# Ignaciagothe/tda-eeg-audio

Hardware: AMD Instinct MI355X
Metric: windows/sec end-to-end (dist->Rips H0/H1->Wasserstein), 47-ch EEG (higher is better)
Workload: dtype f64; 1 GPU; configs[4]+configs[2]: 1416 recordings x 5 bands x 15 selected windows = 106200 (EEG 47x250 f64, audio 250 f64) window pairs per pass, the whole job; per pair corr->dist->Rips H0/H1 (EEG 47 pts), tau per recording-band, Takens dim 3 sub 2 + Rips (audio, 23..123 pts over the bands), Wasserstein H0+H1, features, per-recording reductions; one all-gather of the (1416, 5x48) rows per pass; windows_per_pass=106200, windows_per_gpu_per_pass=106200, input_bytes_per_gpu=10195200000, batches_per_pass=1, windows_per_batch=106200, parallelism=recordings dealt over 1 rank(s), one all-gather per pass, batches_in_flight=3, hip_graph=True, batches_rerun_with_full_ladder=0

## Files before the change

### tda_eeg_audio_amd/csrc/rips.hip

```cpp
#include "common.h"
#include "corr_dist_dev.h"
#include <stdlib.h>

#ifndef CLOUD_NB
#define CLOUD_NB 8192
#endif
#ifndef NARROW_NT
#define NARROW_NT 512
#endif
#ifndef NARROW_WAVES
#define NARROW_WAVES 6
#endif
#if defined(TDA_PROFILE) && !defined(TDA_PROFILE_STOPS_ONLY)
#define NARROW_NB (NARROW_NT == 384 ? 1536 : 1024)
#else
#define NARROW_NB (NARROW_NT == 384 ? 1536 : 2048)
#endif
#define NARROW_EMAX 7626
#define NT_MAX 512
#define RANK_NONE 0x7fffu

#ifdef TDA_PROFILE
__device__ unsigned long long g_prof[48];
#ifdef TDA_PROFILE_STOPS_ONLY
#define PROF_BEGIN() do {} while (0)
#define PROF_RESUME() do {} while (0)
#define PROF_MARK(i) do {} while (0)
#define PROF_COUNT(i, v) do {} while (0)
#define PROF_FLUSH() do {} while (0)
#else
__shared__ unsigned long long prof_lds[48];
#define PROF_BEGIN()                                                       \
    if (threadIdx.x < 48) prof_lds[threadIdx.x] = 0ull;                    \
    __syncthreads();                                                       \
    unsigned long long prof_t0 = clock64()
#define PROF_RESUME() unsigned long long prof_t0 = clock64()
#define PROF_MARK(i)                                                       \
    do {                                                                   \
        unsigned long long prof_t1 = clock64();                            \
        if (threadIdx.x == 0) prof_lds[i] += prof_t1 - prof_t0;            \
        prof_t0 = prof_t1;                                                 \
    } while (0)
#define PROF_COUNT(i, v) do { if (threadIdx.x == 0) prof_lds[i] += (unsigned long long)(v); } while (0)
#define PROF_FLUSH()                                                       \
    do {                                                                   \
        __syncthreads();                                                   \
        if (threadIdx.x < 48 && prof_lds[threadIdx.x]) atomicAdd(&g_prof[threadIdx.x], prof_lds[threadIdx.x]); \
    } while (0)
#endif
__device__ int g_stop_after;
extern "C" __attribute__((visibility("default"))) int tda_profile_stop_after(int n)
{
    return hipMemcpyToSymbol(HIP_SYMBOL(g_stop_after), &n, sizeof(int)) != hipSuccess;
}
#define PROF_STOP(n, cleanup) do { if (g_stop_after == (n)) { cleanup; return; } } while (0)
#define PROF_STOPC(n, cleanup) do { if (g_stop_after == (n) + 100 * prof_chunk) { cleanup; return; } } while (0)
extern "C" __attribute__((visibility("default"))) int tda_profile_read(unsigned long long* out, int reset)
{
    if (hipMemcpyFromSymbol(out, HIP_SYMBOL(g_prof), sizeof(unsigned long long) * 48) != hipSuccess) return 1;
    if (reset) {
        unsigned long long z[48] = {0};
        if (hipMemcpyToSymbol(HIP_SYMBOL(g_prof), z, sizeof(z)) != hipSuccess) return 1;
    }
    return 0;
}
#else
#define PROF_BEGIN() do {} while (0)
#define PROF_RESUME() do {} while (0)
#define PROF_MARK(i) do {} while (0)
#define PROF_COUNT(i, v) do {} while (0)
#define PROF_FLUSH() do {} while (0)
// ... 203 lines not shown
#pragma unroll 4
    for (int e = tid; e < E; e += NT) {
        const u32 b = rank[e];
        u32 r = RANK_NONE;
        if (b != 0xffffu) {
            const u32 k = key32[e];
            const int lo = b ? (int)cur16[b - 1] : 0, hi = (int)cur16[b];
            int c = 0;
            for (int j = lo; j < hi; ++j) {
                const u32 m = members[j];
                const u32 km = key32[m];
                c += (km < k || (km == k && m < (u32)e)) ? 1 : 0;
            }
            r = (u32)(lo + c);
        }
        rank[e] = (u16)r;
    }
    __syncthreads();
#pragma unroll 4
    for (int e = tid; e < E; e += NT) {
        const u32 r = rank[e];
        if (r != RANK_NONE) {
            ord[r] = (u16)edge_ab(e);
            if (WANT_KEYS) skey[r] = key32[e];
        }
    }
    __syncthreads();
    return Ev;
}

#if defined(TDA_PROFILE) && !defined(TDA_PROFILE_STOPS_ONLY)
#define NARROW_LDS ((160 * 1024 / 3 / 1280) * 1280 - 384)
#else
#define NARROW_LDS ((160 * 1024 / 3 / 1280) * 1280)
#endif
#define NARROW_PMAX 124
#define NARROW_DIM 3
#ifdef TDA_DEBUG_PTS
#define NL_GUARD 16
#else
#define NL_GUARD 0
#endif
#define NL_A16(x) (((x) + 15) & ~15)
struct NL {
    static constexpr int E = NARROW_EMAX;
    static constexpr int RANK = 0;
    static constexpr int PSI = NL_A16(2 * E) + NL_GUARD;
    static constexpr int MEMBERS = NL_A16(4 * E);
    static constexpr int CURSOR = NL_A16(MEMBERS + 2 * E);
    static constexpr int RSCR = CURSOR + 2 * NARROW_NB;
    static constexpr int TOTAL = NARROW_LDS;
    static constexpr int AUX = TOTAL - NL_GUARD - NL_A16(NARROW_PMAX * NARROW_DIM * 8);
    static constexpr int MISC = AUX - NL_GUARD - NL_A16(8752 + 8 * 32);
    static constexpr int REGION = MISC - NL_GUARD - PSI;
    static_assert(RSCR + 720 <= AUX - NL_GUARD, "the ranking arrays must end in front of the points");
    static_assert(MEMBERS >= 4 * (E + 1) && CURSOR >= MEMBERS + 2 * (E + 3), "room for the walk's padding (rank_edges_narrow)");
    static_assert(REGION >= 2 * E + 8 * 512, "the first chunks must fit: class vectors of 2 NT ranks next to the whole of ord");
};

template <int NT, int NB>
__device__ __forceinline__ int rank_edges_narrow(const u32* key32, int E, u32 teff, u32 kmin, u16* members, u32* cursor, int* wsum,
                                                 u16* rank, u16* ord)
{
    static_assert(NB % (2 * NT) == 0, "every thread scans whole words");
    static_assert(NB <= 0x8000, "bucket indices are parked in 16 bits, 0xffff = beyond the threshold");
    constexpr int WPT = NB / NT / 2;
    constexpr int EPT = 2 * ((NARROW_EMAX + 2 * NT - 1) / (2 * NT));
    const int tid = threadIdx.x, lane = tid & 63, wave = tid >> 6;
    Bucketer bk;
    bk.dmin = sortable_f32(kmin);
    bk.top = (float)(NB - 1);
    bk.scale = bk.top / (sortable_f32(teff) - bk.dmin);
    for (int i = tid; i < NB / 2; i += NT) cursor[i] = 0u;
    __syncthreads();
    u32 rk[EPT / 2];
#pragma unroll
    for (int i = 0; i < EPT; ++i) {
        const int e = tid + i * NT;
        u32 b = 0xffffu;
        if (e < E) {
            const u32 k = key32[e];
            if (k <= teff) { b = (u32)bk(k); atomicAdd(&cursor[b >> 1], 1u << (16 * (b & 1))); }
        }
        if (i & 1) rk[i >> 1] |= b << 16; else rk[i >> 1] = b;
    }
    __syncthreads();
    {
        u32 w[WPT];
        int s = 0;
#pragma unroll
        for (int i = 0; i < WPT; ++i) {
            const u32 x = cursor[tid * WPT + i];
            const int c0 = (int)(x & 0xffffu), c1 = (int)(x >> 16);
            w[i] = (u32)s | ((u32)(s + c0) << 16);
            s += c0 + c1;
        }
        const int incl = wave_incl_scan_i32(s);
        if (lane == 63) wsum[wave] = incl;
        __syncthreads();
        int basep = incl - s;
        for (int q = 0; q < wave; ++q) basep += wsum[q];
        const u32 add = (u32)basep * 0x00010001u;
#pragma unroll
        for (int i = 0; i < WPT; ++i) cursor[tid * WPT + i] = w[i] + add;
        if (tid == NT - 1) {
            const int total = basep + s;
            members[total] = (u16)NARROW_EMAX; members[total + 1] = (u16)NARROW_EMAX; members[total + 2] = (u16)NARROW_EMAX;
            const_cast<u32*>(key32)[NARROW_EMAX] = 0xffffffffu;
        }
    }
    __syncthreads();
#pragma unroll
    for (int i = 0; i < EPT; ++i) {
        const u32 b = i & 1 ? rk[i >> 1] >> 16 : rk[i >> 1] & 0xffffu;
        if (b != 0xffffu) {
            const int sh = 16 * (int)(b & 1u);
            const u32 old = atomicAdd(&cursor[b >> 1], 1u << sh);
            members[(old >> sh) & 0xffffu] = (u16)(tid + i * NT);
        }
    }
    __syncthreads();
    const u16* cur16 = reinterpret_cast<const u16*>(cursor);
    const int Ev = uni((int)cur16[NB - 1]);
#pragma unroll
    for (int i = 0; i < EPT; ++i) {
        const u32 e = (u32)(tid + i * NT);
        const u32 b = i & 1 ? rk[i >> 1] >> 16 : rk[i >> 1] & 0xffffu;
        u32 r = RANK_NONE;
        if (b != 0xffffu) {
            const u32 k = key32[e];
            const u64 me = ((u64)k << 32) | e;
            const int lo = b ? (int)cur16[b - 1] : 0, hi = (int)cur16[b];
            int c = 0;
            for (int j = lo; j < hi; j += 4) {
                u32 m[4], km[4];
#pragma unroll
                for (int t = 0; t < 4; ++t) m[t] = (u32)members[j + t];
#pragma unroll
                for (int t = 0; t < 4; ++t) km[t] = key32[m[t]];
#pragma unroll
                for (int t = 0; t < 4; ++t) c += ((((u64)km[t] << 32) | m[t]) < me) ? 1 : 0;
            }
            r = (u32)(lo + c);
        }
        if (i & 1) rk[i >> 1] = (rk[i >> 1] & 0xffffu) | (r << 16); else rk[i >> 1] = (rk[i >> 1] & 0xffff0000u) | r;
    }
    __syncthreads();
#pragma unroll
    for (int i = 0; i < EPT; ++i) {
        const int e = tid + i * NT;
        if (e < E) {
            const u32 r = i & 1 ? rk[i >> 1] >> 16 : rk[i >> 1] & 0xffffu;
            rank[e] = (u16)r;
            if (r != RANK_NONE) ord[r] = (u16)edge_ab(e);
        }
    }
    __syncthreads();
    return Ev;
}

struct RipsOut {
    double* h0; int h0_cap; int* h0_cnt;
    double* h1; int h1_cap; int* h1_cnt;
    int* status;
    int* retry_list = nullptr;
};

struct RipsLayout {
    int off_members;
    int off_rank, off_ord, off_aux, off_misc;
    int total;
    int off_psi, psi_bytes, off_cursor, off_rscr;
    int guard[5], n_guard;
};

#define TDA_WIN_LDS_GUARD 0x100
#ifndef TDA_SOLO_PRIO
#define TDA_SOLO_PRIO 3
#endif
#define TDA_SOLO_BEGIN() __builtin_amdgcn_s_setprio(TDA_SOLO_PRIO)
#define TDA_SOLO_END() __builtin_amdgcn_s_setprio(0)

#define TDA_POLL_LIMIT (1 << 16)
#ifndef TDA_TURN_SLEEP
#define TDA_TURN_SLEEP 4
#endif
#ifdef TDA_DEBUG_PTS
__device__ int g_fault;
extern "C" __attribute__((visibility("default"))) int tda_debug_inject(int what)
{
    return hipMemcpyToSymbol(HIP_SYMBOL(g_fault), &what, sizeof(int)) != hipSuccess;
}
#define TDA_FAULT(n) (g_fault == (n))
#else
#define TDA_FAULT(n) false
#endif
#ifdef TDA_DEBUG_PTS
#define GUARD_BYTES 16
__device__ __forceinline__ void guard_write(unsigned char* smem, const RipsLayout& L)
{
    if ((int)threadIdx.x < 4 * L.n_guard) reinterpret_cast<u32*>(smem + L.guard[threadIdx.x >> 2] - GUARD_BYTES)[threadIdx.x & 3] = 0xC0FFEE00u + threadIdx.x;
    __syncthreads();
}
__device__ __forceinline__ int guard_check(unsigned char* smem, const RipsLayout& L)
{
    __syncthreads();
    bool bad = false;
    if ((int)threadIdx.x < 4 * L.n_guard) bad = reinterpret_cast<u32*>(smem + L.guard[threadIdx.x >> 2] - GUARD_BYTES)[threadIdx.x & 3] != 0xC0FFEE00u + threadIdx.x;
    return __syncthreads_or(bad ? 1 : 0) ? TDA_WIN_LDS_GUARD : 0;
}
#else
#define GUARD_BYTES 0
__device__ __forceinline__ void guard_write(unsigned char*, const RipsLayout&) {}
__device__ __forceinline__ int guard_check(unsigned char*, const RipsLayout&) { return 0; }
#endif

#define MISC_COMP 0
#define MISC_CAND 512
#define MISC_WV (512 + 128)
#define MISC_MIN (512 + 192)
#define MISC_DONE (512 + 208)
#define MISC_SORTCNT (512 + 224)
#define MISC_SHARED (MISC_DONE + NT_MAX)
#define MISC_CKEY (MISC_SHARED + 96)
#define MISC_LIST MISC_CKEY
#define MISC_LIST_BYTES (4 * NT_MAX + 1280)
#define MISC_ADJ (MISC_LIST + MISC_LIST_BYTES)
#define MISC_ADJC (MISC_ADJ + 128 * 16)
#define MISC_BRANK (MISC_ADJC + 128 * 16)
#define MISC_BYTES(ncls) (MISC_BRANK + 8 * (ncls))

template <int NT, int NVW, int W, typename WT, bool NARROW, class KEYFN>
__device__ __forceinline__ void rips_sweep(int n, int E, int Ev, const u16* rank, const u16* ord, Psi<W, WT>* psi, int psi_bytes,
                           unsigned char* misc, KEYFN keyfn, double* h0, int h0_cap, double* h1, int h1_cap,
                           int& out_k0, int& out_k1, int& out_status)
{
    static_assert(!NARROW || W == 1, "the narrow layout is the point-cloud first pass");
    int psi_cap = 0;
    const int tid0 = threadIdx.x;
    const int lane0 = tid0 & 63, wave = uni(tid0 >> 6);
    int* brank = reinterpret_cast<int*>(misc + MISC_BRANK);
    u64* cand = reinterpret_cast<u64*>(misc + MISC_CAND);
    unsigned char* done = misc + MISC_DONE;
    SweepShared* shared = reinterpret_cast<SweepShared*>(misc + MISC_SHARED);
    u64* adj = reinterpret_cast<u64*>(misc + MISC_ADJ);
    constexpr int WB = 8 * (int)sizeof(WT);
    float* bkey = reinterpret_cast<float*>(misc + MISC_BRANK + 4 * WB * W);
    u64* adjc = reinterpret_cast<u64*>(misc + MISC_ADJC);

    if constexpr (!NARROW) for (int e = tid0; e < E; e += NT) psi[e] = pzero<W, WT>();
    for (int i = tid0; i < WB * W; i += NT) { brank[i] = -1; bkey[i] = 0.f; }
    for (int i = tid0; i < 256; i += NT) { adj[i] = 0ull; adjc[i] = 0ull; }
    if (tid0 == 0) {
        u32* lc = reinterpret_cast<u32*>(misc + MISC_MIN);
        lc[0] = 0u; lc[1] = 0xffffffffu; lc[2] = 0u;
        lc[3] = 0u;
        shared->status = 0;
    }
    if (tid0 < 16) {
        reinterpret_cast<u32*>(misc + MISC_WV)[tid0] = 0u;
        cand[tid0] = 0ull;
    }
    __syncthreads();

    WgVote vote{reinterpret_cast<u32*>(misc + MISC_WV), 0};
    WT alive[W];
#pragma unroll
    for (int c = 0; c < W; ++c) alive[c] = 0;
    int k0 = 0, k1 = 0, merges = 0, status = 0;
    int compA = lane0, compB = lane0 + 64;

    int clen = NT;
    int ordcls = 0;
    int cov_next = tid0;
#ifdef TDA_PROFILE
    int prof_rneed = 0, prof_chunk = -1;
#endif
    PROF_RESUME();
    for (int r0 = 0; r0 < Ev && !status; r0 += clen) {
        int tid = tid0;
        LAUNDER(tid);
        const int lane = tid & 63;
        clen = NT;
        PROF_MARK(15);
#ifdef TDA_PROFILE
        ++prof_chunk;
#endif
        PROF_COUNT(23, 1);
        const int r = r0 + tid;
        const bool valid = r < Ev;
        int a = 1, b = 0;
        if (valid) { const u32 pk = ord[r]; a = (int)(pk >> 8); b = (int)(pk & 255u); }
        const int tab = tri2(a) + b;
        const int slot = NARROW ? r : tab;
        if constexpr (NARROW) {
            psi_cap = (psi_bytes - 2 * (E - r0)) >> 2;
            if (r < psi_cap) psi[r] = pzero<W, WT>();
        }
        u64 M[NVW], M0[NVW];
        u64 Aj[NVW], Bj[NVW];
#pragma unroll
        for (int w = 0; w < NVW; ++w) { M[w] = 0; M0[w] = 0; Aj[w] = 0; Bj[w] = 0; }
        if (valid) {
#pragma unroll
            for (int w = 0; w < NVW; ++w) { Aj[w] = adj[2 * a + w]; Bj[w] = adj[2 * b + w]; M0[w] = Aj[w] & Bj[w]; }
        }
        {
            volatile u32* turn = reinterpret_cast<volatile u32*>(misc + MISC_MIN) + 2;
            if (wave > 0) {
                int trips = 0;
                for (;;) {
                    const u32 t = (u32)uni((int)*turn);
                    if (t >= (u32)wave) break;
                    if (++trips > TDA_POLL_LIMIT) { if (lane == 0) turn[1] = 1u; break; }
                    if (t + 1u < (u32)wave) __builtin_amdgcn_s_sleep(TDA_TURN_SLEEP); else __builtin_amdgcn_s_sleep(0);
                }
            }
            __builtin_amdgcn_fence(__ATOMIC_ACQUIRE, "workgroup");
            if (valid) {
#pragma unroll
                for (int w = 0; w < NVW; ++w) M[w] = (Aj[w] | adjc[2 * a + w]) & (Bj[w] | adjc[2 * b + w]);
                atomicOr(reinterpret_cast<unsigned long long*>(&adjc[2 * a + (b >> 6)]), 1ull << (b & 63));
                atomicOr(reinterpret_cast<unsigned long long*>(&adjc[2 * b + (a >> 6)]), 1ull << (a & 63));
            }
            LDS_ORDER();
            if (lane == 0 && !(TDA_FAULT(1) && wave == 3)) *turn = (u32)wave + 1u;
        }
        if (valid) {
            const int ta0 = tri2(a), tb0 = tri2(b);
#pragma unroll
            for (int w = 0; w < NVW; ++w) {
                u64 cc = (Aj[w] | adjc[2 * a + w]) & (Bj[w] | adjc[2 * b + w]) & ~M[w];
                while (cc) {
                    const int v0 = 64 * w + __builtin_ctzll(cc); cc &= cc - 1ull;
                    const bool ok1 = cc != 0ull; const int v1 = ok1 ? 64 * w + __builtin_ctzll(cc) : v0; cc &= cc - 1ull;
                    const int t0 = tri2(v0), t1 = tri2(v1);
                    const u32 xa0 = rank[v0 < a ? ta0 + v0 : t0 + a], xb0 = rank[v0 < b ? tb0 + v0 : t0 + b];
                    const u32 xa1 = rank[v1 < a ? ta0 + v1 : t1 + a], xb1 = rank[v1 < b ? tb0 + v1 : t1 + b];
                    if ((int)(xa0 > xb0 ? xa0 : xb0) < r) M[w] |= 1ull << (v0 & 63);
                    if (ok1 && (int)(xa1 > xb1 ? xa1 : xb1) < r) M[w] |= 1ull << (v1 & 63);
                }
            }
        }
// ... 191 lines not shown
        PROF_MARK(22);
        PROF_STOPC(13, out_k0 = k0; out_k1 = k1; out_status = 0);
        clen = uni(offs[19]);
        if (clen == 0) status |= TDA_WIN_CLASS_OVERFLOW;
        if (clen < NT) PROF_COUNT(14, 1);
        bool mrg = is_cand && ((mbal[wave] >> lane) & 1ull);
        bool birth = is_cand && !mrg && tid < clen;
        bool row = mrg && mykey != 0.0f;
        const u64 below = (1ull << lane) - 1ull;
        const int bpre = offs[wave] + __builtin_popcountll(__ballot(birth) & below);
        const int rpre = offs[8 + wave] + __builtin_popcountll(__ballot(row) & below);
        btot = uni(offs[16]);
        const int rtot = uni(offs[17]), mtot = uni(offs[18]);
        if (!status) {
            if (row) {
                const int pos = k0 + rpre;
                if (pos < h0_cap) { h0[2 * pos] = 0.0; h0[2 * pos + 1] = (double)mykey; }
            }
            k0 += rtot; merges += mtot;
            if (birth) {
                const int idx = (int)freebits[bpre];
                const int cw = idx / WB, bit = idx & (WB - 1);
                Psi<W, WT> nv = pzero<W, WT>();
#pragma unroll
                for (int c = 0; c < W; ++c)
                    if (c == cw) nv.w[c] = ((WT)1 << bit);
                if (!NARROW || r < psi_cap) psi[slot] = nv;
                brank[idx] = r;
                bkey[idx] = mykey;
            }
            if (W == 1 && wave == 0 && btot > 0) {
                const int nal = __builtin_popcountll((u64)alive[0]);
                if (lane >= nal && lane < nal + btot) ordcls = (int)freebits[lane - nal];
            }
            int left = btot;
#pragma unroll
            for (int c = 0; c < W; ++c) {
                const u64 f_ = (u64)(WT)~alive[c];
                const int pc = __builtin_popcountll(f_);
                if (left >= pc) { alive[c] = (WT)~(WT)0; left -= pc; }
                else if (left > 0) {
                    int lo = 0, hi = 63;
                    while (lo < hi) {
                        const int mid = (lo + hi) >> 1;
                        if (__builtin_popcountll(f_ & ((2ull << mid) - 1ull)) >= left) hi = mid; else lo = mid + 1;
                    }
                    alive[c] |= (WT)(f_ & ((2ull << lo) - 1ull));
                    left = 0;
                }
            }
        }
        }
        if (status) break;
        PROF_MARK(5);
        PROF_STOPC(14, out_k0 = k0; out_k1 = k1; out_status = 0);
        bool quiet = btot == 0;
#pragma unroll
        for (int c = 0; c < W; ++c) quiet = quiet && alive[c] == 0;
        u32* lcnt = reinterpret_cast<u32*>(misc + MISC_MIN);
        if (quiet) PROF_COUNT(24, 1);
#ifdef TDA_PROFILE
        if (!quiet) prof_rneed = r0 + clen;
#endif
        if constexpr (NARROW) {
            if (!quiet && r0 + NT > psi_cap) { status |= TDA_WIN_CLASS_OVERFLOW; break; }
        }
        if (!quiet) {
        const bool apparent = valid && many != 0 && tid < clen;
        bool pending = apparent;
        Psi<W, WT> base = pzero<W, WT>();
        const int s1 = NARROW ? q1 + r0 : d1, s2 = NARROW ? q2 + r0 : d2;
        if (apparent && q1 < 0 && q2 < 0) {
            base = pxor(psi[s1], psi[s2]);
            psi[slot] = base;
            pending = false;
        }
        volatile unsigned char* vdone = done;
        LDS_ORDER();
        if (!pending) vdone[tid] = 1;
#ifdef TDA_PROFILE
#ifndef TDA_PROFILE_STOPS_ONLY
        if (pending) atomicAdd(&prof_lds[33], 1ull);
#endif
        PROF_COUNT(34, 1);
#endif
        int idle_trips = 0;
        while (__ballot(pending)) {
            PROF_COUNT(32, 1);
            bool ready = false;
            if (pending) ready = (q1 < 0 || vdone[q1]) && (q2 < 0 || vdone[q2]);
            const u64 rbal = __ballot(ready);
            __builtin_amdgcn_fence(__ATOMIC_ACQUIRE, "workgroup");
            if (ready) {
                base = pxor(psi[s1], psi[s2]);
                psi[slot] = base;
                LDS_ORDER();
                vdone[tid] = 1;
                pending = false;
            }
            if (!rbal) {
                if (++idle_trips > TDA_POLL_LIMIT) {
                    if (lane == 0) reinterpret_cast<volatile u32*>(misc + MISC_MIN)[3] = 1u;
                    if (pending) vdone[tid] = 1;
                    break;
                }
                __builtin_amdgcn_s_sleep(1);
            }
        }
        __syncthreads();
        PROF_MARK(6);
        PROF_STOPC(15, out_k0 = k0; out_k1 = k1; out_status = 0);
        u32 m0, m1, m2 = 0u, m3 = 0u;
        {
            u64 rem[NVW];
#pragma unroll
            for (int w = 0; w < NVW; ++w) rem[w] = 0ull;
            if (apparent) {
                u64 comp[NVW];
// ... 414 lines not shown
                    for (int j = 0; j < 4; ++j) {
                        const int jj = j0 + j < nk ? j0 + j : j0;
                        kc[j] = j0 + j < nk ? *reinterpret_cast<const u32*>(list + ES * jj) : 0xffffffffu;
#pragma unroll
                        for (int c = 0; c < W; ++c) kw[j].w[c] = *reinterpret_cast<const WT*>(list + ES * jj + 4 + c * (int)sizeof(WT));
                    }
#pragma unroll 4
                    for (int rr = tid; rr < (r0 + clen < Ev ? r0 + clen : Ev); rr += NT) {
                        const int e = NARROW ? rr : edge_flat(ord[rr]);
                        Psi<W, WT> p = psi[e];
                        bool changed = false;
#pragma unroll
                        for (int j = 0; j < 4; ++j) {
                            if (kc[j] == 0xffffffffu) continue;
                            const int jcw = (int)(kc[j] >> 8), jbit = (int)(kc[j] & 255u);
                            WT sel = 0;
#pragma unroll
                            for (int c = 0; c < W; ++c)
                                if (c == jcw) sel = (p.w[c] >> jbit) & (WT)1;
                            if (sel) { p = pxor(p, kw[j]); changed = true; }
                        }
                        if (changed) psi[e] = p;
                    }
                }
            }
            PROF_MARK(19);
            PROF_STOPC(19, out_k0 = k0; out_k1 = k1; out_status = 0);
            if (complete && !more) break;
            if (++list_rounds > 4 * NT) { status |= TDA_WIN_CLASS_OVERFLOW; break; }
            __syncthreads();
        }
        }
        if (valid && tid < clen) {
            atomicOr(reinterpret_cast<unsigned long long*>(&adj[2 * a + (b >> 6)]), 1ull << (b & 63));
            atomicOr(reinterpret_cast<unsigned long long*>(&adj[2 * b + (a >> 6)]), 1ull << (a & 63));
        }
        if (tid < 256) adjc[tid] = 0ull;
        if (tid == 0) {
            lcnt[0] = 0u; lcnt[1] = 0xffffffffu; lcnt[2] = 0u; shared->clen = 0x7fffffff;
            if (lcnt[3]) shared->status = TDA_WIN_NOT_CONVERGED;
        }
        __syncthreads();
        if (uni(shared->status) & TDA_WIN_NOT_CONVERGED) { status |= TDA_WIN_NOT_CONVERGED; break; }
        if (quiet) {
            const int from = r0 + clen;
            bool covered = true;
            int rr = (NT & (NT - 1)) == 0 ? from + ((tid - from) & (NT - 1)) : from + (((tid - from) % NT) + NT) % NT;
            rr = rr > cov_next ? rr : cov_next;
            while (rr < Ev) {
                const u32 pk = ord[rr];
                const int ea = (int)(pk >> 8), eb = (int)(pk & 255u);
                u64 common = adj[2 * ea] & adj[2 * eb];
                if (NVW == 2) common |= adj[2 * ea + 1] & adj[2 * eb + 1];
                if (common == 0ull) { covered = false; break; }
                rr += NT;
            }
            cov_next = rr;
            {
                const u32 wmin = wave_min_u32_dpp(covered ? 0x7fffffffu : (u32)rr);
                if (lane == 0 && wmin != 0x7fffffffu) atomicMin(reinterpret_cast<unsigned int*>(&shared->clen), wmin);
            }
            __syncthreads();
            const int ru = uni(shared->clen);
            if (ru >= Ev) { PROF_COUNT(25, 1); PROF_MARK(7); break; }
            if (ru > from) {
                for (int r2 = from + tid; r2 < ru; r2 += NT) {
                    const u32 pk = ord[r2];
                    const int ea = (int)(pk >> 8), eb = (int)(pk & 255u);
                    atomicOr(reinterpret_cast<unsigned long long*>(&adj[2 * ea + (eb >> 6)]), 1ull << (eb & 63));
                    atomicOr(reinterpret_cast<unsigned long long*>(&adj[2 * eb + (ea >> 6)]), 1ull << (ea & 63));
                    if constexpr (NARROW) { if (r2 < ((psi_bytes - 2 * (E - ru)) >> 2)) psi[r2] = pzero<W, WT>(); }
                }
                PROF_COUNT(35, ru - from);
                clen = ru - r0;
                __syncthreads();
            }
        }
        PROF_MARK(7);
        PROF_STOPC(20, out_k0 = k0; out_k1 = k1; out_status = 0);
    }
#ifdef TDA_PROFILE
    PROF_COUNT(36, prof_rneed > 4096 ? 1 : 0); PROF_COUNT(37, prof_rneed > 4608 ? 1 : 0); PROF_COUNT(38, prof_rneed > 5120 ? 1 : 0);
    PROF_COUNT(39, prof_rneed); PROF_COUNT(40, Ev);
#endif
    const int ncomp = n - merges;
    for (int i = 0; i < ncomp; ++i) {
        if (k0 < h0_cap && tid0 == 0) { h0[2 * k0] = 0.0; h0[2 * k0 + 1] = (double)INFINITY; }
        ++k0;
    }
#pragma unroll
    for (int c = 0; c < W; ++c) {
        u64 al = (u64)alive[c];
        while (al) {
            const int bit = __builtin_ctzll(al);
            al &= al - 1;
            if (k1 < h1_cap && tid0 == 0) { h1[2 * k1] = (double)bkey[WB * c + bit]; h1[2 * k1 + 1] = (double)INFINITY; }
            ++k1;
        }
    }
    if (k1 > h1_cap) status |= TDA_WIN_H1_TRUNCATED;
    out_k0 = k0; out_k1 = k1; out_status = status;
}


#define TOT_NW 128
#define TOT_SLOTS 8
#define TOT_SLOT_WORDS ((size_t)8128 * TOT_NW)
#define RETRY_GRID 512
#define RETRY_GRID_WIDE 64

template <int NT, class KEYFN>
__device__ __forceinline__ void rips_sweep_total(int n, int E, int Ev, const u16* rank, const u16* ord, float* bkey, unsigned char* misc,
                                 u64* __restrict__ psi_g, KEYFN keyfn, double* h0, int h0_cap, double* h1, int h1_cap,
                                 int& out_k0, int& out_k1, int& out_status)
{
    constexpr int NWV = NT / 64;
    const int tid = threadIdx.x, lane = tid & 63, wave = uni(tid >> 6);
// ... 113 lines not shown
    }
    int status = 0;
    const int ncomp = n - merges;
    for (int i = 0; i < ncomp; ++i) {
        if (k0 < h0_cap && tid == 0) { h0[2 * k0] = 0.0; h0[2 * k0 + 1] = (double)INFINITY; }
        ++k0;
    }
    for (int c = 0; c < nborn; ++c)
        if ((alivebit[c >> 5] >> (c & 31)) & 1u) {
            if (k1 < h1_cap && tid == 0) { h1[2 * k1] = (double)bkey[c]; h1[2 * k1 + 1] = (double)INFINITY; }
            ++k1;
        }
    if (k1 > h1_cap) status |= TDA_WIN_H1_TRUNCATED;
    out_k0 = k0; out_k1 = k1; out_status = status;
}

struct KeyFromLds {
    const u32* skey;
    __device__ __forceinline__ float operator()(int r, int, int) const { return sortable_f32(skey[r]); }
};

template <int NT, int NVW, int W, typename WT, bool TOTAL = false>
__device__ __forceinline__ void rips_dm_rest(unsigned char* smem, const int win, int n, float thresh, const u32* vmax, u32 kmin_thread,
                             const RipsLayout& L, const RipsOut& out, u64* psi_g = nullptr)
{
    const int tid = threadIdx.x;
    const int E = tri2(n);
    u32* key32 = reinterpret_cast<u32*>(smem);
    u16* members = reinterpret_cast<u16*>(smem + L.off_members);
    Psi<W, WT>* psi = reinterpret_cast<Psi<W, WT>*>(smem);
    u16* rank = reinterpret_cast<u16*>(smem + L.off_rank);
    u16* ord = reinterpret_cast<u16*>(smem + L.off_ord);
    u32* skey = reinterpret_cast<u32*>(smem + L.off_aux);
    unsigned char* misc = smem + L.off_misc;
    u32* red = reinterpret_cast<u32*>(misc + MISC_MIN);
    u32* cursor = reinterpret_cast<u32*>(misc + MISC_SORTCNT);
    int* wsum = reinterpret_cast<int*>(misc + MISC_WV);
    const u32 tkey = f32_sortable(thresh);
    u32 teff, kmin;
    PROF_RESUME();
    effective_threshold<NT>(n, tkey, vmax, kmin_thread, red, teff, kmin);
    PROF_STOP(1, if (tid == 0) { out.h0_cnt[win] = 0; out.h1_cnt[win] = 0; out.status[win] = 0; });
    const int Ev = rank_edges<NT, (NVW == 1 ? 2048 : 8192), true>(key32, E, teff, kmin, members, cursor, wsum, rank, ord, skey);
    PROF_MARK(1);
    PROF_STOP(2, if (tid == 0) { out.h0_cnt[win] = 0; out.h1_cnt[win] = 0; out.status[win] = 0; });
    guard_write(smem, L);
    int k0, k1, st;
    KeyFromLds kf{skey};
    if constexpr (TOTAL)
        rips_sweep_total<NT>(n, E, Ev, rank, ord, reinterpret_cast<float*>(smem), misc, psi_g, kf,
                             out.h0 + (size_t)win * out.h0_cap * 2, out.h0_cap,
                             out.h1 + (size_t)win * out.h1_cap * 2, out.h1_cap, k0, k1, st);
    else
    rips_sweep<NT, NVW, W, WT, false>(n, E, Ev, rank, ord, psi, 0, misc, kf,
                       out.h0 + (size_t)win * out.h0_cap * 2, out.h0_cap,
                       out.h1 + (size_t)win * out.h1_cap * 2, out.h1_cap, k0, k1, st);
    st |= guard_check(smem, L);
    PROF_MARK(3);
    PROF_COUNT(8, 1);
    PROF_COUNT(9, E);
    PROF_FLUSH();
    if (tid == 0) { out.h0_cnt[win] = k0; out.h1_cnt[win] = k1; out.status[win] = st; }
}

template <int NT, int NVW, int W, typename WT, bool TOTAL = false>
__device__ __forceinline__ void rips_dm_window(unsigned char* smem, const int win, const double* __restrict__ dm, int n, float thresh,
                               int symmetrise, const RipsLayout& L, const RipsOut& out, u64* psi_g = nullptr)
{
    const int tid = threadIdx.x;
    const int E = tri2(n);
    u32* key32 = reinterpret_cast<u32*>(smem);
    unsigned char* misc = smem + L.off_misc;
    PROF_BEGIN();
    const double* D = dm + (size_t)win * n * n;
    u32* vmax = reinterpret_cast<u32*>(misc + MISC_COMP);
    if (tid < 128) vmax[tid] = 0u;
    __syncthreads();
    u32 kmin_thread = 0xffffffffu;
    for (int e = tid; e < E; e += NT) {
        const int a = edge_row(e), b = e - tri2(a);
        double v;
        if (symmetrise) {
            v = (D[(size_t)a * n + b] + D[(size_t)b * n + a]) / 2.0;
            if (v < 0.0) v = 0.0;
        } else {
            v = D[(size_t)b * n + a];
        }
        const u32 sk = f32_sortable((float)v);
        key32[e] = sk;
        kmin_thread = sk < kmin_thread ? sk : kmin_thread;
        atomicMax(&vmax[a], sk);
        atomicMax(&vmax[b], sk);
    }
    __syncthreads();
    PROF_MARK(0);
    rips_dm_rest<NT, NVW, W, WT, TOTAL>(smem, win, n, thresh, vmax, kmin_thread, L, out, psi_g);
}

#ifdef TDA_DEBUG_PTS
__device__ double g_dbg[2048];
extern "C" __attribute__((visibility("default"))) int tda_debug_read(double* out)
{
    return hipMemcpyFromSymbol(out, HIP_SYMBOL(g_dbg), sizeof(double) * 2048) != hipSuccess;
}
#endif
struct KeyFromPts {
    const double* pts;
// ... 166 lines not shown
    __syncthreads();
    if (normalise) {
        if ((tid >> 6) < dim) {
            const int k = tid >> 6, l = tid & 63;
            double mn = INFINITY, mx = -INFINITY;
            for (int i = l; i < P; i += 64) {
                const double v = pts[i * dim + k];
                mn = v < mn ? v : mn;
                mx = v > mx ? v : mx;
            }
            mn = wave_min_f64(mn);
            mx = wave_max_f64(mx);
            if (l == 0) { double rg = mx - mn; if (rg == 0.0) rg = 1.0; mm[2 * k] = mn; mm[2 * k + 1] = rg; }
        }
        __syncthreads();
        for (int idx = tid; idx < P * dim; idx += NT) {
            const int k = idx % dim;
            pts[idx] = (pts[idx] - mm[2 * k]) / mm[2 * k + 1];
        }
        __syncthreads();
    }
#ifdef TDA_DEBUG_PTS
    for (int idx = tid; idx < P * dim; idx += NT) g_dbg[idx] = pts[idx];
#endif
    const int E = tri2(P);
    const u32 tkey = f32_sortable(thresh);
    KeyFromPts kf{pts, dim};
    u32* vmax = reinterpret_cast<u32*>(rscr + MISC_COMP);
    u32* cursor = reinterpret_cast<u32*>(smem + (NARROW ? NL::CURSOR : L.off_cursor));
    int* wsum = reinterpret_cast<int*>(rscr + MISC_WV);
    if (tid < 128) vmax[tid] = 0u;
    double* nrm = reinterpret_cast<double*>(cursor);
    if (tid < P) nrm[tid] = KeyFromPtsTab::norm2(pts + tid * dim, dim);
    __syncthreads();
    const KeyFromPtsTab kft{pts, nrm, dim};
    u32 kmin_thread = 0xffffffffu;
    u32 ab_next = edge_ab(tid);
    for (int e = tid; e < E; e += NT) {
        const u32 ab = ab_next;
        ab_next = edge_ab(e + NT);
        const int a = (int)(ab >> 8), b = (int)(ab & 255u);
        const u32 sk = f32_sortable(kft(0, a, b));
        key32[e] = sk;
        kmin_thread = sk < kmin_thread ? sk : kmin_thread;
        atomicMax(&vmax[b], sk);
    }
    __syncthreads();
    row_maxima<NT>(key32, vmax, P);
    __syncthreads();
    u32 teff, kmin;
    effective_threshold<NT>(P, tkey, vmax, kmin_thread, red, teff, kmin);
    PROF_MARK(0);
    PROF_STOP(1, if (tid == 0) { out.h0_cnt[win] = 0; out.h1_cnt[win] = 0; out.status[win] = 0; });
    int Ev;
    if constexpr (NARROW) {
        ord = reinterpret_cast<u16*>(smem + NL::PSI + NL::REGION) - E;
        Ev = rank_edges_narrow<NT, NARROW_NB>(key32, E, teff, kmin, members, cursor, wsum, rank, ord);
    }
    else Ev = rank_edges<NT, CLOUD_NB, false>(key32, E, teff, kmin, members, cursor, wsum, rank, ord, nullptr);
    PROF_MARK(1);
    PROF_STOP(2, if (tid == 0) { out.h0_cnt[win] = 0; out.h1_cnt[win] = 0; out.status[win] = 0; });
    guard_write(smem, L);
    int k0, k1, st;
    if constexpr (TOTAL)
        rips_sweep_total<NT>(P, E, Ev, rank, ord, reinterpret_cast<float*>(smem), misc, psi_g, kf, h0, out.h0_cap, h1, out.h1_cap, k0, k1, st);
    else if (P <= 64)
        rips_sweep<NT, 1, W, WT, NARROW>(P, E, Ev, rank, ord, psi, NL::REGION, misc, kf, h0, out.h0_cap, h1, out.h1_cap, k0, k1, st);
    else
        rips_sweep<NT, 2, W, WT, NARROW>(P, E, Ev, rank, ord, psi, NL::REGION, misc, kf, h0, out.h0_cap, h1, out.h1_cap, k0, k1, st);
    st |= guard_check(smem, L);
    PROF_MARK(3);
    PROF_COUNT(8, 1);
    PROF_COUNT(9, E);
    PROF_FLUSH();
#ifdef TDA_DEBUG_PTS
    __syncthreads();
    for (int idx = tid; idx < P * dim; idx += NT) g_dbg[1024 + idx] = pts[idx];
#endif
    if (tid == 0) { out.h0_cnt[win] = k0; out.h1_cnt[win] = k1; out.status[win] = st; }
}

#ifndef CLOUD_WAVES
#define CLOUD_WAVES 4
#endif
template <int NT, int W, typename WT, bool RETRY, bool NARROW = false>
__global__ void __launch_bounds__(NT, RETRY ? 2 : (NARROW ? NARROW_WAVES : CLOUD_WAVES))
rips_cloud_kernel(const double* __restrict__ src, const int* __restrict__ tau_or_npts, int n_win,
                  int n_t_or_pcap, int dim, int subsample, int mode, int normalise, float thresh,
                  RipsLayout L, int p_max, int* __restrict__ n_points, RipsOut out,
                  unsigned long long* __restrict__ span, unsigned long long* __restrict__ retry_ctr)
{
    extern __shared__ __attribute__((aligned(16))) unsigned char smem[];
    if (span && blockIdx.x == 0 && threadIdx.x == 0)
        atomicExch(&span[0], wall_clock64());
    if constexpr (!RETRY) {
        if ((int)blockIdx.x < n_win)
            rips_cloud_window<NT, W, WT, NARROW>(smem, (int)blockIdx.x, src, tau_or_npts, n_t_or_pcap, dim, subsample, mode,
                                                 normalise, thresh, L, p_max, n_points, out);
    } else {
        RETRY_SCAN_BEGIN(NT, out, n_win)
            if (retry_ctr && threadIdx.x == 0) atomicAdd(retry_ctr + 1, 1ull);
            rips_cloud_window<NT, W, WT, false>(smem, win, src, tau_or_npts, n_t_or_pcap, dim, subsample, mode, normalise,
                                                thresh, L, p_max, n_points, out);
        RETRY_SCAN_END()
    }
    if (span && threadIdx.x == 0) {
        const unsigned long long now = wall_clock64();
        if (atomicAdd(&span[1], 1ull) == (unsigned long long)gridDim.x - 1ull) {
            const unsigned long long first = atomicAdd(&span[0], 0ull);
            atomicAdd(&span[2], now - first);
            atomicAdd(&span[3], 1ull);
            atomicExch(&span[1], 0ull);
        }
    }
}

template <int NT>
__global__ void __launch_bounds__(NT, 2)
rips_dm_total_kernel(const double* __restrict__ dm, int n_win, int n, float thresh, int symmetrise, RipsLayout L,
                     RipsOut out, u64* __restrict__ scratch, unsigned long long* __restrict__ retry_ctr)
{
    extern __shared__ __attribute__((aligned(16))) unsigned char smem[];
// ... 507 lines not shown
```

Baseline: 4.419 million windows/s.

## Rank only the first NARROW_REFINE edges exactly in the narrow Rips pass

```diff
diff --git a/tda_eeg_audio_amd/csrc/rips.hip b/tda_eeg_audio_amd/csrc/rips.hip
--- a/tda_eeg_audio_amd/csrc/rips.hip
+++ b/tda_eeg_audio_amd/csrc/rips.hip
@@ -17,6 +17,9 @@
 #define NARROW_NB (NARROW_NT == 384 ? 1536 : 2048)
 #endif
 #define NARROW_EMAX 7626
+#ifndef NARROW_REFINE
+#define NARROW_REFINE 5120
+#endif
 #define NT_MAX 512
 #define RANK_NONE 0x7fffu
 
@@ -326,20 +329,25 @@
     static constexpr int TOTAL = NARROW_LDS;
     static constexpr int AUX = TOTAL - NL_GUARD - NL_A16(NARROW_PMAX * NARROW_DIM * 8);
     static constexpr int MISC = AUX - NL_GUARD - NL_A16(8752 + 8 * 32);
-    static constexpr int REGION = MISC - NL_GUARD - PSI;
+    static constexpr int BSTART_BITS = NL_A16((E - NARROW_REFINE + 512 + 7) / 8) * 8;
+    static constexpr int BSTART = MISC - NL_GUARD - BSTART_BITS / 8;
+    static constexpr int REGION = BSTART - PSI;
     static_assert(RSCR + 720 <= AUX - NL_GUARD, "the ranking arrays must end in front of the points");
     static_assert(MEMBERS >= 4 * (E + 1) && CURSOR >= MEMBERS + 2 * (E + 3), "room for the walk's padding (rank_edges_narrow)");
     static_assert(REGION >= 2 * E + 8 * 512, "the first chunks must fit: class vectors of 2 NT ranks next to the whole of ord");
+    static_assert(BSTART + BSTART_BITS / 8 <= CURSOR, "the bits lie clear of the cursors they are made from");
 };
 
 template <int NT, int NB>
 __device__ __forceinline__ int rank_edges_narrow(const u32* key32, int E, u32 teff, u32 kmin, u16* members, u32* cursor, int* wsum,
-                                                 u16* rank, u16* ord)
+                                                 u16* rank, u16* ord, u32* bstart, int& r_exact)
 {
     static_assert(NB % (2 * NT) == 0, "every thread scans whole words");
     static_assert(NB <= 0x8000, "bucket indices are parked in 16 bits, 0xffff = beyond the threshold");
+    static_assert(NARROW_REFINE < 0x2000, "13 bits for a member and for a rank");
     constexpr int WPT = NB / NT / 2;
     constexpr int EPT = 2 * ((NARROW_EMAX + 2 * NT - 1) / (2 * NT));
+    constexpr int PPT = (NARROW_REFINE + NT - 1) / NT;
     const int tid = threadIdx.x, lane = tid & 63, wave = tid >> 6;
     Bucketer bk;
     bk.dmin = sortable_f32(kmin);
@@ -376,48 +384,61 @@
         for (int q = 0; q < wave; ++q) basep += wsum[q];
         const u32 add = (u32)basep * 0x00010001u;
 #pragma unroll
-        for (int i = 0; i < WPT; ++i) cursor[tid * WPT + i] = w[i] + add;
+        for (int i = 0; i < WPT; ++i) {
+            cursor[tid * WPT + i] = w[i] + add;
+            const int s0 = basep + (int)(w[i] & 0xffffu), s1 = basep + (int)(w[i] >> 16);
+            const int s2 = basep + (i + 1 < WPT ? (int)(w[(i + 1) % WPT] & 0xffffu) : s);
+            if (s0 <= NARROW_REFINE && NARROW_REFINE < s1) wsum[NT / 64] = s0;
+            if (s1 <= NARROW_REFINE && NARROW_REFINE < s2) wsum[NT / 64] = s1;
+        }
         if (tid == NT - 1) {
             const int total = basep + s;
             members[total] = (u16)NARROW_EMAX; members[total + 1] = (u16)NARROW_EMAX; members[total + 2] = (u16)NARROW_EMAX;
             const_cast<u32*>(key32)[NARROW_EMAX] = 0xffffffffu;
+            if (total <= NARROW_REFINE) wsum[NT / 64] = total;
         }
     }
     __syncthreads();
 #pragma unroll
     for (int i = 0; i < EPT; ++i) {
         const u32 b = i & 1 ? rk[i >> 1] >> 16 : rk[i >> 1] & 0xffffu;
+        u32 pos = RANK_NONE;
         if (b != 0xffffu) {
             const int sh = 16 * (int)(b & 1u);
             const u32 old = atomicAdd(&cursor[b >> 1], 1u << sh);
-            members[(old >> sh) & 0xffffu] = (u16)(tid + i * NT);
-        }
+            pos = (old >> sh) & 0xffffu;
+            members[pos] = (u16)(tid + i * NT);
+        }
+        if (i & 1) rk[i >> 1] = (rk[i >> 1] & 0xffffu) | (pos << 16); else rk[i >> 1] = (rk[i >> 1] & 0xffff0000u) | pos;
     }
     __syncthreads();
     const u16* cur16 = reinterpret_cast<const u16*>(cursor);
     const int Ev = uni((int)cur16[NB - 1]);
-#pragma unroll
-    for (int i = 0; i < EPT; ++i) {
-        const u32 e = (u32)(tid + i * NT);
-        const u32 b = i & 1 ? rk[i >> 1] >> 16 : rk[i >> 1] & 0xffffu;
-        u32 r = RANK_NONE;
-        if (b != 0xffffu) {
+    const int rx = uni(wsum[NT / 64]);
+    u32 pr[PPT];
+#pragma unroll
+    for (int i = 0; i < PPT; ++i) {
+        const int j = tid + i * NT;
+        u32 v = 0u;
+        if (j < rx) {
+            const u32 e = (u32)members[j];
             const u32 k = key32[e];
+            const u32 b = (u32)bk(k);
             const u64 me = ((u64)k << 32) | e;
             const int lo = b ? (int)cur16[b - 1] : 0, hi = (int)cur16[b];
             int c = 0;
-            for (int j = lo; j < hi; j += 4) {
+            for (int jj = lo; jj < hi; jj += 4) {
                 u32 m[4], km[4];
 #pragma unroll
-                for (int t = 0; t < 4; ++t) m[t] = (u32)members[j + t];
+                for (int t = 0; t < 4; ++t) m[t] = (u32)members[jj + t];
 #pragma unroll
                 for (int t = 0; t < 4; ++t) km[t] = key32[m[t]];
 #pragma unroll
                 for (int t = 0; t < 4; ++t) c += ((((u64)km[t] << 32) | m[t]) < me) ? 1 : 0;
             }
-            r = (u32)(lo + c);
-        }
-        if (i & 1) rk[i >> 1] = (rk[i >> 1] & 0xffffu) | (r << 16); else rk[i >> 1] = (rk[i >> 1] & 0xffff0000u) | r;
+            v = e | ((u32)(lo + c) << 16);
+        }
+        pr[i] = v;
     }
     __syncthreads();
 #pragma unroll
@@ -425,11 +446,34 @@
         const int e = tid + i * NT;
         if (e < E) {
             const u32 r = i & 1 ? rk[i >> 1] >> 16 : rk[i >> 1] & 0xffffu;
+            if (r >= (u32)rx) {
+                rank[e] = (u16)r;
+                if (r != RANK_NONE) ord[r] = (u16)edge_ab(e);
+            }
+        }
+    }
+#pragma unroll
+    for (int i = 0; i < PPT; ++i) {
+        if (tid + i * NT < rx) {
+            const u32 e = pr[i] & 0xffffu, r = pr[i] >> 16;
             rank[e] = (u16)r;
-            if (r != RANK_NONE) ord[r] = (u16)edge_ab(e);
-        }
-    }
-    __syncthreads();
+            ord[r] = (u16)edge_ab((int)e);
+        }
+    }
+    if (rx < Ev) {
+        for (int i = tid; i < NL::BSTART_BITS / 32; i += NT) bstart[i] = 0u;
+        __syncthreads();
+        int prev = tid ? (int)cur16[2 * WPT * tid - 1] : 0;
+#pragma unroll
+        for (int i = 0; i < 2 * WPT; ++i) {
+            const int end = (int)cur16[2 * WPT * tid + i];
+            const int q = prev - rx;
+            if (end > prev && q >= 0 && q < NL::BSTART_BITS) atomicOr(&bstart[q >> 5], 1u << (q & 31));
+            prev = end;
+        }
+    }
+    __syncthreads();
+    r_exact = rx;
     return Ev;
 }
 
@@ -505,11 +549,12 @@
 #define MISC_BYTES(ncls) (MISC_BRANK + 8 * (ncls))
 
 template <int NT, int NVW, int W, typename WT, bool NARROW, class KEYFN>
-__device__ __forceinline__ void rips_sweep(int n, int E, int Ev, const u16* rank, const u16* ord, Psi<W, WT>* psi, int psi_bytes,
-                           unsigned char* misc, KEYFN keyfn, double* h0, int h0_cap, double* h1, int h1_cap,
+__device__ __forceinline__ void rips_sweep(int n, int E, int Ev, int r_exact, const u16* rank, const u16* ord, Psi<W, WT>* psi,
+                           int psi_bytes, unsigned char* misc, KEYFN keyfn, double* h0, int h0_cap, double* h1, int h1_cap,
                            int& out_k0, int& out_k1, int& out_status)
 {
     static_assert(!NARROW || W == 1, "the narrow layout is the point-cloud first pass");
+    const int Rx = NARROW ? r_exact : Ev;
     int psi_cap = 0;
     const int tid0 = threadIdx.x;
     const int lane0 = tid0 & 63, wave = uni(tid0 >> 6);
@@ -562,7 +607,7 @@
 #endif
         PROF_COUNT(23, 1);
         const int r = r0 + tid;
-        const bool valid = r < Ev;
+        const bool valid = r < Rx;
         int a = 1, b = 0;
         if (valid) { const u32 pk = ord[r]; a = (int)(pk >> 8); b = (int)(pk & 255u); }
         const int tab = tri2(a) + b;
@@ -860,6 +905,7 @@
         }
         }
         if (status) break;
+        if constexpr (NARROW) clen = clen < Rx - r0 ? clen : Rx - r0;
         PROF_MARK(5);
         PROF_STOPC(14, out_k0 = k0; out_k1 = k1; out_status = 0);
         bool quiet = btot == 0;
@@ -871,7 +917,7 @@
         if (!quiet) prof_rneed = r0 + clen;
 #endif
         if constexpr (NARROW) {
-            if (!quiet && r0 + NT > psi_cap) { status |= TDA_WIN_CLASS_OVERFLOW; break; }
+            if (!quiet && (r0 + NT > psi_cap || r0 >= Rx)) { status |= TDA_WIN_CLASS_OVERFLOW; break; }
         }
         if (!quiet) {
         const bool apparent = valid && many != 0 && tid < clen;
@@ -1392,7 +1438,27 @@
                 const int ea = (int)(pk >> 8), eb = (int)(pk & 255u);
                 u64 common = adj[2 * ea] & adj[2 * eb];
                 if (NVW == 2) common |= adj[2 * ea + 1] & adj[2 * eb + 1];
-                if (common == 0ull) { covered = false; break; }
+                if (common == 0ull) {
+                    bool shorter = false;
+                    if constexpr (NARROW) {
+                        const int q = rr - Rx;
+                        if (from >= Rx && q < NL::BSTART_BITS) {
+                            const u32* bstart = reinterpret_cast<const u32*>(reinterpret_cast<const unsigned char*>(psi) + psi_bytes);
+                            int wd = q >> 5;
+                            u32 bits = bstart[wd] & (0xffffffffu >> (31 - (q & 31)));
+                            while (bits == 0u && wd > 0) bits = bstart[--wd];
+                            const int s = bits ? Rx + 32 * wd + 31 - __builtin_clz(bits) : 0;
+                            const int ta = tri2(ea), tb = tri2(eb);
+                            for (int v = 0; v < n && !shorter; ++v) {
+                                const int tv = tri2(v);
+                                const u32 xa = v == ea ? RANK_NONE : rank[v < ea ? ta + v : tv + ea];
+                                const u32 xb = v == eb ? RANK_NONE : rank[v < eb ? tb + v : tv + eb];
+                                shorter = (int)(xa > xb ? xa : xb) < s;
+                            }
+                        }
+                    }
+                    if (!shorter) { covered = false; break; }
+                }
                 rr += NT;
             }
             cov_next = rr;
@@ -1401,8 +1467,14 @@
                 if (lane == 0 && wmin != 0x7fffffffu) atomicMin(reinterpret_cast<unsigned int*>(&shared->clen), wmin);
             }
             __syncthreads();
-            const int ru = uni(shared->clen);
+            int ru = uni(shared->clen);
             if (ru >= Ev) { PROF_COUNT(25, 1); PROF_MARK(7); break; }
+            if constexpr (NARROW) {
+                if (ru >= Rx) {
+                    if (from >= Rx) { status |= TDA_WIN_CLASS_OVERFLOW; break; }
+                    ru = Rx;
+                }
+            }
             if (ru > from) {
                 for (int r2 = from + tid; r2 < ru; r2 += NT) {
                     const u32 pk = ord[r2];
@@ -1622,7 +1694,7 @@
                              out.h0 + (size_t)win * out.h0_cap * 2, out.h0_cap,
                              out.h1 + (size_t)win * out.h1_cap * 2, out.h1_cap, k0, k1, st);
     else
-    rips_sweep<NT, NVW, W, WT, false>(n, E, Ev, rank, ord, psi, 0, misc, kf,
+    rips_sweep<NT, NVW, W, WT, false>(n, E, Ev, Ev, rank, ord, psi, 0, misc, kf,
                        out.h0 + (size_t)win * out.h0_cap * 2, out.h0_cap,
                        out.h1 + (size_t)win * out.h1_cap * 2, out.h1_cap, k0, k1, st);
     st |= guard_check(smem, L);
@@ -1895,12 +1967,13 @@
     effective_threshold<NT>(P, tkey, vmax, kmin_thread, red, teff, kmin);
     PROF_MARK(0);
     PROF_STOP(1, if (tid == 0) { out.h0_cnt[win] = 0; out.h1_cnt[win] = 0; out.status[win] = 0; });
-    int Ev;
+    int Ev, r_exact;
     if constexpr (NARROW) {
         ord = reinterpret_cast<u16*>(smem + NL::PSI + NL::REGION) - E;
-        Ev = rank_edges_narrow<NT, NARROW_NB>(key32, E, teff, kmin, members, cursor, wsum, rank, ord);
-    }
-    else Ev = rank_edges<NT, CLOUD_NB, false>(key32, E, teff, kmin, members, cursor, wsum, rank, ord, nullptr);
+        Ev = rank_edges_narrow<NT, NARROW_NB>(key32, E, teff, kmin, members, cursor, wsum, rank, ord,
+                                              reinterpret_cast<u32*>(smem + NL::BSTART), r_exact);
+    }
+    else { Ev = rank_edges<NT, CLOUD_NB, false>(key32, E, teff, kmin, members, cursor, wsum, rank, ord, nullptr); r_exact = Ev; }
     PROF_MARK(1);
     PROF_STOP(2, if (tid == 0) { out.h0_cnt[win] = 0; out.h1_cnt[win] = 0; out.status[win] = 0; });
     guard_write(smem, L);
@@ -1908,9 +1981,9 @@
     if constexpr (TOTAL)
         rips_sweep_total<NT>(P, E, Ev, rank, ord, reinterpret_cast<float*>(smem), misc, psi_g, kf, h0, out.h0_cap, h1, out.h1_cap, k0, k1, st);
     else if (P <= 64)
-        rips_sweep<NT, 1, W, WT, NARROW>(P, E, Ev, rank, ord, psi, NL::REGION, misc, kf, h0, out.h0_cap, h1, out.h1_cap, k0, k1, st);
+        rips_sweep<NT, 1, W, WT, NARROW>(P, E, Ev, r_exact, rank, ord, psi, NL::REGION, misc, kf, h0, out.h0_cap, h1, out.h1_cap, k0, k1, st);
     else
-        rips_sweep<NT, 2, W, WT, NARROW>(P, E, Ev, rank, ord, psi, NL::REGION, misc, kf, h0, out.h0_cap, h1, out.h1_cap, k0, k1, st);
+        rips_sweep<NT, 2, W, WT, NARROW>(P, E, Ev, r_exact, rank, ord, psi, NL::REGION, misc, kf, h0, out.h0_cap, h1, out.h1_cap, k0, k1, st);
     st |= guard_check(smem, L);
     PROF_MARK(3);
     PROF_COUNT(8, 1);
```

Measured after the change: 4.426 million windows/s (median of 6 runs). About the same (+0.2%).
